# serviceberry3/weiner_slamit_v2

Hardware: AMD Instinct MI355X
Metric: frames/sec ORB extract+match @640x480x8lvl (higher is better)
Workload: dtype u8; 1 GPU; BASELINE configs[1]: 640x480 8-level ORB extract (1000 features, FAST 20/7) + brute-force 256-bit Hamming best/second match vs the stream's previous frame; 256 independent streams per GPU per step; distinct_frame_pairs_per_gpu=16, parallelism=streams sharded over 1 GPU(s), no data-path collective

## Files before the change

weiner_slamit_v2_amd/csrc/orb_kernels.hip:

```cpp
#include <hip/hip_runtime.h>
#include <stdint.h>

#include <algorithm>

#include "orb_types.h"
#include "slamit_math.h"
#include "../../include/slamit.h"
#include "../../include/slamit_orb_pattern.h"

#define WAVE 64

__global__ __launch_bounds__(256) void resize_level_kernel(
    const uint8_t* __restrict__ src, int sw, int sh, size_t sstride, size_t sframe,
    uint8_t* __restrict__ dst, int dw, int dh, size_t dstride, size_t dframe,
    const int* __restrict__ xofs, const short* __restrict__ ialpha,
    const int* __restrict__ yofs, const short* __restrict__ ibeta) {
    const int x4 = (blockIdx.x * 64 + (threadIdx.x & 63)) * 4;
    const int y = blockIdx.y * 4 + (threadIdx.x >> 6);
    const int f = blockIdx.z;
    if (x4 >= dw || y >= dh) return;
    const uint8_t* S = src + (size_t)f * sframe;
    int sy = yofs[y];
    int sy0 = min(max(sy, 0), sh - 1), sy1 = min(max(sy + 1, 0), sh - 1);
    const uint8_t* S0 = S + (size_t)sy0 * sstride;
// ... 752 lines not shown
            int lx = order & 63, ly = (order >> 6) & 63, cell = order >> 12;
            int ci = (int)__umulhi((unsigned)cell, inv_cols), cj = cell - ci * nCols;
            int x = cj * wCell + lx, y = ci * hCell + ly;
            int r = (int)((float)x / hX);
            r = min(r, nIni - 1);
            if (valid) XY[k] = (uint32_t)x | ((uint32_t)y << 16);
            if (FD) {
                Box16 b = box0[r];
                int path = 0;
                for (int d = 0; d < FD; ++d) {
                    int mx, my;
                    const int q = box_quadrant(b, x, y, &mx, &my);
                    b = child_box(b, q);
                    path = path * 4 + q;
                }
                if (valid) ND[k] = (uint16_t)((r << 8) | path);
                const int bin = valid ? r * HS + (HS - (1 << (2 * FD))) + path : -1;
                const int prev = __shfl_up(bin, 1);
                const bool head = lane == 0 || bin != prev;
                const unsigned long long heads = __ballot(head);
                if (head && bin >= 0) {
                    const unsigned long long rest = (heads >> lane) >> 1;
                    atomicAdd(&hist[bin], rest ? (int)__builtin_ctzll(rest) + 1 : 64 - lane);
                }
            } else {
                if (valid) ND[k] = (uint16_t)r;
                for (int q = 0; q < nIni; ++q) {
                    const unsigned long long m = __ballot(valid && r == q);
                    if (m && lane == (int)__builtin_ctzll(m)) atomicAdd(&cnt0[q], (int)__popcll(m));
                }
            }
            }
        }
    }
    __syncthreads();
    for (int d = FD - 1; d >= 1; --d) {
        const int off = ((4 << (2 * d)) - 4) / 3 - (1 << (2 * d)), offc = off + (1 << (2 * d)), per = 1 << (2 * d);
        for (int e = tid; e < nIni * per; e += NT) {
            const int r = e >> (2 * d), pth = e & (per - 1);
            const int* c = &hist[r * HS + offc + 4 * pth];
            hist[r * HS + off + pth] = (c[0] + c[1]) + (c[2] + c[3]);
        }
        __syncthreads();
    }
    if (tid == 0) {
        int m = 0, dropped = 0;
        for (int i = 0; i < nIni; ++i) {
            if (FD) cnt0[i] = (hist[i * HS] + hist[i * HS + 1]) + (hist[i * HS + 2] + hist[i * HS + 3]);
            if (cnt0[i] > 0) { scanbuf[i] = m; box0[m] = box0[i]; cnt0[m] = cnt0[i]; ncode0[m] = i << 16; ++m; }
            else { scanbuf[i] = -1; dropped = 1; }
        }
        s_n = m; s_flag = dropped;
    }
    __syncthreads();
    if (s_flag && !FD) {
        for (int k = tid; k < n_keys; k += NT) ND[k] = (uint16_t)scanbuf[ND[k]];
        __syncthreads();
    }

    int cur = 0;
    int n = s_n;
    bool finish = false, careful = false;
    bool tabled = FD > 0;
    int depth_done = 0;
    auto label_keys = [&]() {
        for (int e = tid; e < nIni * HS; e += NT) hist[e] = -1;
        if (tid < ORB_MAX_ROOTS) scanbuf[tid] = -1;
        __syncthreads();
        for (int i = tid; i < n; i += NT) {
            const int c = ncode0[cur * cap + i], r = c >> 16, d = (c >> 12) & 15, pth = c & 4095;
            if (d == 0) scanbuf[r] = i;
            else hist[r * HS + ((4 << (2 * d)) - 4) / 3 - (1 << (2 * d)) + pth] = i;
        }
        __syncthreads();
        for (int k = tid; k < n_keys; k += NT) {
            const int lab = ND[k], r = lab >> 8, pth = lab & 255;
            int node = scanbuf[r];
            for (int d = 1; d <= FD; ++d) {
                const int v = hist[r * HS + ((4 << (2 * d)) - 4) / 3 - (1 << (2 * d)) + (pth >> (2 * (FD - d)))];
                node = v >= 0 ? v : node;
            }
            ND[k] = (uint16_t)node;
        }
        __syncthreads();
    };
    OD_STAMP(0);
    while (!finish) {
        const int prevSize = n;
#ifdef OCT_DIAG
        ++od_pass;
#endif
        const bool tpass = tabled && !careful && depth_done < FD;
        if (tabled && !tpass) { label_keys(); tabled = false; }
        if (tpass) {
            for (int e = tid; e < 4 * n; e += NT) {
                const int i = e >> 2, c = ncode0[cur * cap + i], r = c >> 16, d = (c >> 12) & 15, pth = c & 4095;
                childcnt[e] = cnt0[cur * cap + i] > 1 ? hist[r * HS + ((4 << (2 * (d + 1))) - 4) / 3 - (1 << (2 * (d + 1))) + 4 * pth + (e & 3)] : 0;
            }
        } else {
        for (int i = tid; i < 4 * n; i += NT) childcnt[i] = 0;
        __syncthreads();
        for (int k = tid; k < n_keys; k += NT) {
            int nd = ND[k];
            if (cnt0[cur * cap + nd] > 1) {
                uint32_t xy = XY[k];
                int mx, my;
                int q = box_quadrant(box0[cur * cap + nd], xy & 0xFFFF, xy >> 16, &mx, &my);
                atomicAdd(&childcnt[nd * 4 + q], 1);
                ND[k] = (uint16_t)(nd | ((q + 1) << 12));
            }
        }
        }
        __syncthreads();
        OD_STAMP(1);

        int kproc;
        if (!careful) {
            kproc = -1;
        } else {
            for (int i = tid >> 6; i < n; i += NT / 64) {
                const int ci_ = cnt0[cur * cap + i];
                int r = -1;
                if (ci_ > 1) {
                    r = 0;
                    for (int j0 = 0; j0 < n; j0 += 64) {
                        const int j = j0 + (tid & 63);
                        const int cj_ = j < n ? cnt0[cur * cap + j] : 0;
                        r += (int)__popcll(__ballot((cj_ > 1) && (cj_ > ci_ || (cj_ == ci_ && j < i))));
                    }
                    if ((tid & 63) == 0) sorted[r] = i;
                }
                if ((tid & 63) == 0) rankv[i] = r;
            }
            if (tid == 0) s_expand = 0;
            __syncthreads();
            int local = 0;
            for (int i = tid; i < n; i += NT) local += cnt0[cur * cap + i] > 1;
            if (local) atomicAdd(&s_expand, local);
            __syncthreads();
            const int m = s_expand;
            for (int s = tid; s < m; s += NT) {
                int i = sorted[s];
                const int* cc = &childcnt[i * 4];
                scanbuf[s] = (cc[0] > 0) + (cc[1] > 0) + (cc[2] > 0) + (cc[3] > 0) - 1;
            }
            if (tid == 0) s_k = m;
            __syncthreads();
            block_exclusive_scan<NT>(scanbuf, m, wave_tmp);
            for (int s = tid; s < m; s += NT) {
                int i = sorted[s];
                const int* cc = &childcnt[i * 4];
                int g = (cc[0] > 0) + (cc[1] > 0) + (cc[2] > 0) + (cc[3] > 0) - 1;
                if (n + scanbuf[s] + g >= N) atomicMin(&s_k, s + 1);
            }
            __syncthreads();
            kproc = s_k;
        }

        OD_STAMP(2);
        int nchildslots;
        if (!careful) {
            nchildslots = 4 * n;
            for (int e = tid; e < 4 * n; e += NT) {
                int i = n - 1 - (e >> 2), q = 3 - (e & 3);
                scanbuf[e] = (cnt0[cur * cap + i] > 1) && (childcnt[i * 4 + q] > 0);
            }
            for (int i = tid; i < n; i += NT) scanbuf[4 * n + i] = cnt0[cur * cap + i] <= 1;
        } else {
            nchildslots = 4 * kproc;
            for (int e = tid; e < nchildslots; e += NT) {
                int s = kproc - 1 - (e >> 2), q = 3 - (e & 3);
                scanbuf[e] = childcnt[sorted[s] * 4 + q] > 0;
            }
            for (int i = tid; i < n; i += NT) {
                int r = rankv[i];
                scanbuf[nchildslots + i] = !(r >= 0 && r < kproc);
            }
        }
        __syncthreads();
        const int n_new = block_exclusive_scan<NT>(scanbuf, nchildslots + n, wave_tmp);
        const int nxt = cur ^ 1;
        if (tid == 0) s_expand = 0;
        __syncthreads();
        int local_expand = 0;
        for (int e = tid; e < nchildslots; e += NT) {
            int i, q;
            if (!careful) { i = n - 1 - (e >> 2); q = 3 - (e & 3); }
            else { i = sorted[kproc - 1 - (e >> 2)]; q = 3 - (e & 3); }
            bool split = !careful ? (cnt0[cur * cap + i] > 1) : true;
            int cc = childcnt[i * 4 + q];
            if (split && cc > 0) {
                int pos = scanbuf[e];
                if (pos < cap) {
                    box0[nxt * cap + pos] = child_box(box0[cur * cap + i], q);
                    cnt0[nxt * cap + pos] = cc;
                    if (tpass) { const int c = ncode0[cur * cap + i]; ncode0[nxt * cap + pos] = (c & ~0xFFFF) | ((((c >> 12) & 15) + 1) << 12) | (4 * (c & 4095) + q); }
                }
                local_expand += cc > 1;
            }
        }
        for (int i = tid; i < n; i += NT) {
            bool stays = !careful ? (cnt0[cur * cap + i] <= 1) : !(rankv[i] >= 0 && rankv[i] < kproc);
            if (stays) {
                int pos = scanbuf[nchildslots + i];
                if (pos < cap) {
                    box0[nxt * cap + pos] = box0[cur * cap + i]; cnt0[nxt * cap + pos] = cnt0[cur * cap + i];
                    if (tpass) ncode0[nxt * cap + pos] = ncode0[cur * cap + i];
                }
            }
        }
        if (local_expand) atomicAdd(&s_expand, local_expand);
        OD_STAMP(3);
        if (!tpass)
        for (int k = tid; k < n_keys; k += NT) {
            const int lab = ND[k];
            const int nd = lab & 4095, q = (lab >> 12) - 1;
            bool split = !careful ? (q >= 0) : (rankv[nd] >= 0 && rankv[nd] < kproc);
            int pos;
            if (split) {
                int e = !careful ? ((n - 1 - nd) * 4 + (3 - q)) : ((kproc - 1 - rankv[nd]) * 4 + (3 - q));
                pos = scanbuf[e];
            } else {
                pos = scanbuf[nchildslots + nd];
            }
            ND[k] = (uint16_t)min(pos, cap - 1);
        }
        __syncthreads();
        const int nToExpand = s_expand;
        cur = nxt;
        n = min(n_new, cap);
        __syncthreads();
        if (n >= N || n == prevSize) finish = true;
        else if (!careful && n + nToExpand * 3 > N) careful = true;
        ++depth_done;
        OD_STAMP(4);
    }
    if (tabled) label_keys();

    for (int i = tid; i < n; i += NT) best[i] = 0ull;
    __syncthreads();
    for (int k = tid; k < n_keys; k += NT) {
        unsigned long long c = K[k];
        unsigned long long packed = (c & 0xFFFFFFFF00000000ull) | (0xFFFFFFFFu - (unsigned)c);
        atomicMax(&best[ND[k]], packed);
    }
    __syncthreads();
    for (int i = tid; i < n; i += NT) {
        unsigned long long b = best[i];
        unsigned order = 0xFFFFFFFFu - (unsigned)b;
        int lx = order & 63, ly = (order >> 6) & 63, cell = order >> 12;
        int ci = cell / L.nCols, cj = cell - ci * L.nCols;
        OrbLevelKp kp;
        kp.x = (int16_t)(cj * L.wCell + lx + ORB_MIN_BORDER);
        kp.y = (int16_t)(ci * L.hCell + ly + ORB_MIN_BORDER);
        kp.response = (float)(unsigned)(b >> 32);
        kp.angle = 0.f; kp.cs = 1.f; kp.sn = 0.f;
        if (i < L.kp_cap) OUT[i] = kp;
    }
    if (tid == 0) *kp_count_out = min(n, L.kp_cap);
#ifdef OCT_DIAG
    OD_STAMP(5);
    if (tid == 0) {
        const int w = blockIdx.y * gridDim.x + blockIdx.x;
        if (w < 4096) { unsigned long long* o = g_oct_ph + 8 * w; for (int k = 0; k < 6; ++k) o[k] = od_ph[k]; o[6] = ((unsigned long long)od_pass << 32) | (unsigned)n_keys; o[7] = od_rt0; o[5] = __builtin_amdgcn_s_memrealtime(); }
    }
#endif
}

template <int OCT_NT>
__global__ __launch_bounds__(OCT_NT) void octree_kernel(
    const OrbLevel* __restrict__ levels, int nlevels,
    const unsigned long long* __restrict__ cand, size_t cand_frame_stride,
    int* __restrict__ cand_count,
    uint32_t* __restrict__ ws_xy, uint16_t* __restrict__ ws_node,
    OrbLevelKp* __restrict__ lkp, size_t kp_frame_stride, int* __restrict__ kp_count,
    int node_cap, int key_cap, int level_override ) {
    extern __shared__ __attribute__((aligned(16))) unsigned char smem[];
    __shared__ int wave_tmp[OCT_NT / 64];
    __shared__ int s_vars[4];
    uint32_t* k_xy = reinterpret_cast<uint32_t*>(smem + orbk_octree_node_bytes(node_cap));
    uint16_t* k_nd = reinterpret_cast<uint16_t*>(k_xy + key_cap);
    const int level = level_override >= 0 ? level_override : blockIdx.y;
    const int frame = blockIdx.x;
    const OrbLevel& L = levels[level];
    const int kidx = frame * nlevels + level;
    const int n_raw = cand_count[kidx * ORB_CC_PAD];
    const int n_keys = min(n_raw, L.cand_cap);
    __syncthreads();
    if (threadIdx.x == 0) { cand_count[kidx * ORB_CC_PAD] = 0; cand_count[kidx * ORB_CC_PAD + 1] = n_raw; }
    const unsigned long long* K = cand + L.cand_off + (size_t)frame * cand_frame_stride;
    OrbLevelKp* OUT = lkp + L.kp_off + (size_t)frame * kp_frame_stride;
    if (n_keys == 0) {
        if (threadIdx.x == 0) kp_count[kidx] = 0;
        return;
    }
    if (n_keys <= key_cap)
        octree_body<OCT_NT, true>(L, K, n_keys, k_xy, k_nd, OUT, &kp_count[kidx], smem, node_cap, wave_tmp, s_vars);
    else
        octree_body<OCT_NT, false>(L, K, n_keys, ws_xy + L.cand_off + (size_t)frame * cand_frame_stride,
                                        ws_node + L.cand_off + (size_t)frame * cand_frame_stride, OUT, &kp_count[kidx], smem,
                                        node_cap, wave_tmp, s_vars);
}

struct DiscTable { signed char uv[64][32]; int n; };
__constant__ DiscTable c_disc;

static DiscTable make_disc() {
    static const int umax[16] = {15, 15, 15, 15, 14, 14, 14, 13, 13, 12, 11, 10, 9, 8, 6, 3};
    DiscTable t;
    for (int l = 0; l < 64; ++l) for (int k = 0; k < 32; ++k) t.uv[l][k] = 0;
    t.n = 0;
    for (int v = -15; v <= 15; ++v)
        for (int u = -umax[v < 0 ? -v : v]; u <= umax[v < 0 ? -v : v]; ++u) {
            t.uv[t.n & 63][2 * (t.n >> 6)] = (signed char)u; t.uv[t.n & 63][2 * (t.n >> 6) + 1] = (signed char)v;
            ++t.n;
        }
    return t;
}

#define IC_KP_PER_WAVE 8
#define IC_R 15
#define IC_ROWS (2 * IC_R + 1)
#define IC_PITCH 32

template <int CTRL>
__device__ __forceinline__ int dpp_i32(int v) { return __builtin_amdgcn_update_dpp(0, v, CTRL, 0xF, 0xF, false); }
__device__ __forceinline__ int wave_sum_i32(int v) {
    v += dpp_i32<0xB1>(v);
    v += dpp_i32<0x4E>(v);
    v += dpp_i32<0x141>(v);
    v += dpp_i32<0x140>(v);
    return __builtin_amdgcn_readlane(v, 0) + __builtin_amdgcn_readlane(v, 16) + __builtin_amdgcn_readlane(v, 32) + __builtin_amdgcn_readlane(v, 48);
}

__global__ __launch_bounds__(256) void ic_angle_kernel(
    const OrbLevel* __restrict__ levels, int nlevels,
    const uint8_t* __restrict__ img0, size_t img0_stride, size_t img0_frame,
    const uint8_t* __restrict__ pyr,
    OrbLevelKp* __restrict__ lkp, size_t kp_frame_stride, const int* __restrict__ kp_count, int xcd_frames, int kblocks) {
    const int lane = threadIdx.x & 63;
    int level, frame, kb;
    if (xcd_frames) {
        const unsigned w = blockIdx.x, k = w >> 3, P = (unsigned)(nlevels * kblocks), fq = k / P, local = k - fq * P;
        frame = (int)(8u * fq + ((w + fq) & 7u));
        if (frame >= xcd_frames) return;
        level = (int)(local / (unsigned)kblocks); kb = (int)(local - (unsigned)level * (unsigned)kblocks);
    } else { level = blockIdx.y; frame = blockIdx.z; kb = blockIdx.x; }
    const OrbLevel& L = levels[level];
    const int count = kp_count[frame * nlevels + level];
    const int i0 = (kb * 4 + (threadIdx.x >> 6)) * IC_KP_PER_WAVE;
    if (i0 >= count) return;
    const uint8_t* src;
    int stride;
    if (level == 0) { src = img0 + (size_t)frame * img0_frame; stride = (int)img0_stride; }
    else { src = pyr + L.plane_off + (size_t)frame * L.plane_bytes; stride = L.stride; }
    __shared__ __attribute__((aligned(16))) uint8_t s_win[4][IC_KP_PER_WAVE][IC_ROWS * IC_PITCH];
    const int wvi = threadIdx.x >> 6;
    OrbLevelKp* kp0 = lkp + L.kp_off + (size_t)frame * kp_frame_stride;
    typedef unsigned ic_u4 __attribute__((ext_vector_type(4), aligned(1)));
    {
        const int lr = min(lane >> 1, IC_ROWS - 1), lc = lane & 1;
        const unsigned loff = __umul24((unsigned)lr, (unsigned)stride) + 16u * (unsigned)lc;
        ic_u4 ld[IC_KP_PER_WAVE];
#pragma unroll
        for (int k = 0; k < IC_KP_PER_WAVE; ++k) {
            const int i = min(i0 + k, count - 1);
            const uint8_t* corner = src + (__umul24((unsigned)(kp0[i].y - IC_R), (unsigned)stride) + (unsigned)(kp0[i].x - IC_R));
            ld[k] = *reinterpret_cast<const ic_u4*>(corner + loff);
        }
#pragma unroll
        for (int k = 0; k < IC_KP_PER_WAVE; ++k)
            if (lane < 2 * IC_ROWS) *reinterpret_cast<uint4*>(&s_win[wvi][k][lr * IC_PITCH + 16 * lc]) = make_uint4(ld[k].x, ld[k].y, ld[k].z, ld[k].w);
    }
    int off[12], wu[12], wv[12];
    {
        const uint4 t0 = *reinterpret_cast<const uint4*>(&c_disc.uv[lane][0]);
        const uint2 t1 = *reinterpret_cast<const uint2*>(&c_disc.uv[lane][16]);
        const uint32_t tw[6] = {t0.x, t0.y, t0.z, t0.w, t1.x, t1.y};
#pragma unroll
        for (int j = 0; j < 12; ++j) {
            const uint32_t pr = tw[j >> 1] >> (16 * (j & 1));
            const int u = (int)(signed char)(pr & 0xFFu), v = (int)(signed char)((pr >> 8) & 0xFFu);
            off[j] = (v + IC_R) * IC_PITCH + (u + IC_R); wu[j] = u; wv[j] = v;
        }
    }
    const float factorPI = (float)(3.14159265358979323846 / 180.f);
    wave_sync_lds();
    int val[IC_KP_PER_WAVE][12];
#pragma unroll
    for (int k = 0; k < IC_KP_PER_WAVE; ++k)
#pragma unroll
        for (int j = 0; j < 12; ++j) val[k][j] = s_win[wvi][k][off[j]];
    int V[2 * IC_KP_PER_WAVE];
#pragma unroll
    for (int k = 0; k < IC_KP_PER_WAVE; ++k) {
        int m10 = 0, m01 = 0;
#pragma unroll
        for (int j = 0; j < 12; ++j) { m10 += __mul24(wu[j], val[k][j]); m01 += __mul24(wv[j], val[k][j]); }
        V[2 * k] = m10; V[2 * k + 1] = m01;
    }
    {
        const bool b0 = lane & 1, b1 = lane & 2, b2 = lane & 4, b3 = lane & 8;
#pragma unroll
        for (int p = 0; p < 8; ++p) { const int a = V[2 * p], b = V[2 * p + 1]; V[p] = (b0 ? b : a) + dpp_i32<0xB1>(b0 ? a : b); }
#pragma unroll
        for (int p = 0; p < 4; ++p) { const int a = V[2 * p], b = V[2 * p + 1]; V[p] = (b1 ? b : a) + dpp_i32<0x4E>(b1 ? a : b); }
#pragma unroll
        for (int p = 0; p < 2; ++p) { const int a = V[2 * p], b = V[2 * p + 1]; V[p] = (b2 ? b : a) + dpp_i32<0x1B>(dpp_i32<0x141>(b2 ? a : b)); }
        { const int a = V[0], b = V[1]; V[0] = (b3 ? b : a) + dpp_i32<0x141>(dpp_i32<0x140>(b3 ? a : b)); }
    }
    __shared__ int s_rows[4][64];
    int* sr = s_rows[threadIdx.x >> 6];
    sr[lane] = V[0];
    wave_sync_lds();
    const int tot = (sr[lane & 15] + sr[(lane & 15) + 16]) + (sr[(lane & 15) + 32] + sr[(lane & 15) + 48]);
    const int my10 = tot, my01 = dpp_i32<0xB1>(tot);
    if (lane < 2 * IC_KP_PER_WAVE && !(lane & 1) && i0 + (lane >> 1) < count) {
        const float ang = slamit_fast_atan2((float)my01, (float)my10);
        float sn, cs;
        slamit_sincosf(ang * factorPI, &sn, &cs);
        OrbLevelKp* kp = kp0 + i0 + (lane >> 1);
        kp->angle = ang; kp->cs = cs; kp->sn = sn;
    }
}

__device__ __forceinline__ int reflect101(int p, int len) {
    p = p < 0 ? -p : p;
    p = p >= len ? 2 * len - 2 - p : p;
    return min(max(p, 0), len - 1);
}


typedef unsigned short blur_us2 __attribute__((ext_vector_type(2)));
__device__ __forceinline__ uint32_t udot2(uint32_t a, uint32_t b, uint32_t c) {
    return __builtin_amdgcn_udot2(__builtin_bit_cast(blur_us2, a), __builtin_bit_cast(blur_us2, b), c, false);
}

__device__ __forceinline__ uint32_t blur_fetch(const uint8_t* S, unsigned sstride, bool whole, int w, int h, int gx0, int row) {
    const unsigned ro = (unsigned)reflect101(row, h) * sstride;
    if (whole) return *reinterpret_cast<const uint32_t*>(S + (ro + (unsigned)gx0));
    if (gx0 >= w + 3) return 0u;
    uint32_t v = 0;
#pragma unroll
    for (int j = 0; j < 4; ++j) v |= (uint32_t)S[ro + (unsigned)reflect101(gx0 + j, w)] << (8 * j);
    return v;
}

struct BlurCol { unsigned a0, a1, sel; };
__device__ __forceinline__ BlurCol blur_col(int g, int w, unsigned ss) {
#define BLUR_SEL(i0, i1, i2, i3) ((unsigned)(i0) | ((unsigned)(i1) << 8) | ((unsigned)(i2) << 16) | ((unsigned)(i3) << 24))
    BlurCol c;
    if (g < 0) { c.a0 = 0u; c.a1 = 4u; c.sel = BLUR_SEL(4, 3, 2, 1); }
    else if (g + 4 <= w) { c.a0 = c.a1 = (unsigned)g; c.sel = BLUR_SEL(0, 1, 2, 3); }
    else if (g < w) {
        const int q = w - g;
        unsigned idx[4];
#pragma unroll
        for (int j = 0; j < 4; ++j) idx[j] = (unsigned)(j < q ? 4 + j : 2 * q + 2 - j);
        c.a0 = (unsigned)(g - 4); c.a1 = (unsigned)g; c.sel = BLUR_SEL(idx[0], idx[1], idx[2], idx[3]);
    } else if (g <= w + 2) {
        const int t = g - w, gb = (w - 4) & ~3;
        unsigned idx[4];
#pragma unroll
        for (int j = 0; j < 4; ++j) idx[j] = j <= 2 - t ? (unsigned)(w - 2 - t - j - gb) : 0x0Cu;
        c.a0 = (unsigned)gb; c.a1 = min((unsigned)gb + 4u, ss - 4u); c.sel = BLUR_SEL(idx[0], idx[1], idx[2], idx[3]);
    } else { c.a0 = c.a1 = 0u; c.sel = BLUR_SEL(0x0C, 0x0C, 0x0C, 0x0C); }
#undef BLUR_SEL
    return c;
}
__device__ __forceinline__ uint32_t blur_fetch2(const uint8_t* S, unsigned ss, int h, int row, const BlurCol c) {
    const unsigned ro = __umul24((unsigned)reflect101(row, h), ss);
    return __builtin_amdgcn_perm(*reinterpret_cast<const uint32_t*>(S + (ro + c.a1)), *reinterpret_cast<const uint32_t*>(S + (ro + c.a0)), c.sel);
}

template <bool INTERIOR>
__device__ __forceinline__ void blur_strip(uint8_t (*in)[72], uint32_t (*rp)[64], const uint8_t* S, const size_t sstride, const bool aligned,
                                           uint8_t* D, const unsigned dstride, const int w, const int h, const int bx, const int by0, const int tid) {
    const int i0 = tid, i1 = tid + 256;
    const bool has1 = i1 < 22 * 18;
    const int r0 = i0 / 18, r1 = i1 / 18;
    const int g0 = bx - 4 + 4 * (i0 - r0 * 18), g1 = bx - 4 + 4 * (i1 - r1 * 18);
    const bool whole0 = aligned && g0 >= 0 && g0 + 4 <= w, whole1 = aligned && g1 >= 0 && g1 + 4 <= w;
    uint32_t* const st0 = reinterpret_cast<uint32_t*>(&in[r0][4 * (i0 - r0 * 18)]);
    uint32_t* const st1 = reinterpret_cast<uint32_t*>(&in[has1 ? r1 : 0][has1 ? 4 * (i1 - r1 * 18) : 0]);
    const unsigned ss = (unsigned)sstride;
    const BlurCol bc0 = blur_col(g0, w, ss), bc1 = blur_col(g1, w, ss);
    uint32_t v0 = INTERIOR ? *reinterpret_cast<const uint32_t*>(S + (__umul24((unsigned)(by0 + r0 - 3), ss) + (unsigned)g0))
                           : aligned ? blur_fetch2(S, ss, h, by0 + r0 - 3, bc0) : blur_fetch(S, ss, whole0, w, h, g0, by0 + r0 - 3);
    uint32_t v1 = !has1 ? 0u : INTERIOR ? *reinterpret_cast<const uint32_t*>(S + (__umul24((unsigned)(by0 + r1 - 3), ss) + (unsigned)g1))
                                        : aligned ? blur_fetch2(S, ss, h, by0 + r1 - 3, bc1) : blur_fetch(S, ss, whole1, w, h, g1, by0 + r1 - 3);
    *st0 = v0;
    if (has1) *st1 = v1;
    __syncthreads();
    const uint32_t TA = 18u | (34u << 8) | (49u << 16) | (55u << 24), TB = 49u | (34u << 8) | (18u << 16);
    const int cy = tid >> 4, cx4 = (tid & 15) * 4;
    const bool odd = cy & 1;
    const uint32_t k0 = odd ? (18u << 16) : (18u | (34u << 16)), k1 = odd ? (34u | (49u << 16)) : (49u | (55u << 16));
    const uint32_t k2 = odd ? (55u | (49u << 16)) : (49u | (34u << 16)), k3 = odd ? (34u | (18u << 16)) : 18u;
#pragma unroll 1
    for (int s = 0; s < BLUR_STEPS; ++s) {
        const int by = by0 + 16 * s;
        const bool more = s + 1 < BLUR_STEPS && (INTERIOR || by + 16 < h);
        if (more) {
            if (INTERIOR) {
                v0 = *reinterpret_cast<const uint32_t*>(S + (__umul24((unsigned)(by + 16 + r0 - 3), ss) + (unsigned)g0));
                if (has1) v1 = *reinterpret_cast<const uint32_t*>(S + (__umul24((unsigned)(by + 16 + r1 - 3), ss) + (unsigned)g1));
            } else {
                if (aligned) {
                    v0 = blur_fetch2(S, ss, h, by + 16 + r0 - 3, bc0);
                    if (has1) v1 = blur_fetch2(S, ss, h, by + 16 + r1 - 3, bc1);
                } else {
                    v0 = blur_fetch(S, ss, whole0, w, h, g0, by + 16 + r0 - 3);
                    if (has1) v1 = blur_fetch(S, ss, whole1, w, h, g1, by + 16 + r1 - 3);
                }
            }
        }
        if (tid < 11 * 16) {
            const int p = tid >> 4, c = (tid & 15) * 4;
            uint32_t o[2][4];
#pragma unroll
            for (int rr = 0; rr < 2; ++rr) {
                const uint32_t* pw = reinterpret_cast<const uint32_t*>(&in[2 * p + rr][c]);
                const uint32_t w0 = pw[0], w1 = pw[1], w2 = pw[2];
                o[rr][0] = __builtin_amdgcn_udot4(__builtin_amdgcn_alignbyte(w2, w1, 1), TB, __builtin_amdgcn_udot4(__builtin_amdgcn_alignbyte(w1, w0, 1), TA, 0u, false), false);
                o[rr][1] = __builtin_amdgcn_udot4(__builtin_amdgcn_alignbyte(w2, w1, 2), TB, __builtin_amdgcn_udot4(__builtin_amdgcn_alignbyte(w1, w0, 2), TA, 0u, false), false);
                o[rr][2] = __builtin_amdgcn_udot4(__builtin_amdgcn_alignbyte(w2, w1, 3), TB, __builtin_amdgcn_udot4(__builtin_amdgcn_alignbyte(w1, w0, 3), TA, 0u, false), false);
                o[rr][3] = __builtin_amdgcn_udot4(w2, TB, __builtin_amdgcn_udot4(w1, TA, 0u, false), false);
            }
            *reinterpret_cast<uint4*>(&rp[p][c]) = make_uint4(o[0][0] | (o[1][0] << 16), o[0][1] | (o[1][1] << 16),
                                                               o[0][2] | (o[1][2] << 16), o[0][3] | (o[1][3] << 16));
        }
        __syncthreads();
        if (more) {
            *st0 = v0;
            if (has1) *st1 = v1;
        }
        if (INTERIOR || (bx + cx4 < w && by + cy < h)) {
            const int pb = cy >> 1;
            const uint4 a0 = *reinterpret_cast<const uint4*>(&rp[pb][cx4]), a1 = *reinterpret_cast<const uint4*>(&rp[pb + 1][cx4]);
            const uint4 a2 = *reinterpret_cast<const uint4*>(&rp[pb + 2][cx4]), a3 = *reinterpret_cast<const uint4*>(&rp[pb + 3][cx4]);
#define BLUR_COL(f) min((udot2(a3.f, k3, udot2(a2.f, k2, udot2(a1.f, k1, udot2(a0.f, k0, 1u << 15)))) >> 16), 255u)
            const uint32_t out = BLUR_COL(x) | (BLUR_COL(y) << 8) | (BLUR_COL(z) << 16) | (BLUR_COL(w) << 24);
#undef BLUR_COL
            *reinterpret_cast<uint32_t*>(D + (__umul24((unsigned)(by + cy), dstride) + (unsigned)(bx + cx4))) = out;
        }
        if (!more) break;
        __syncthreads();
    }
}

__global__ __launch_bounds__(256) void blur_all_kernel(
    const OrbLevel* __restrict__ levels, const uint4* __restrict__ tiles,
    const uint8_t* __restrict__ img0, size_t img0_stride, size_t img0_frame,
    const uint8_t* __restrict__ pyr, uint8_t* __restrict__ blur, unsigned ntiles, unsigned inv_tiles, unsigned total) {
    __shared__ __attribute__((aligned(16))) uint8_t in[22][72];
    __shared__ __attribute__((aligned(16))) uint32_t rp[11][64];
    const int tid = threadIdx.x;
    const unsigned lin = blockIdx.x, per_xcd = (total + 7u) >> 3;
    const unsigned logical = (lin & 7u) * per_xcd + (lin >> 3);
    if (logical >= total) return;
    int frame = (int)__umulhi(logical, inv_tiles);
    if ((unsigned)frame * ntiles > logical) --frame;
    const uint4 tt = tiles[logical - (unsigned)frame * ntiles];
    const int level = (int)tt.x, bx = (int)tt.y, by0 = (int)tt.z;
    const OrbLevel& L = levels[level];
    const int w = L.w, h = L.h;
    const uint8_t* S;
    size_t sstride;
    if (level == 0) { S = img0 + (size_t)frame * img0_frame; sstride = img0_stride; }
    else { S = pyr + L.plane_off + (size_t)frame * L.plane_bytes; sstride = (size_t)L.stride; }
    const bool aligned = ((((uintptr_t)S) | sstride) & 3) == 0;
    uint8_t* D = blur + L.blur_off + (size_t)frame * L.blur_bytes;
    const bool interior = aligned && bx >= 4 && bx + 68 <= w && by0 >= 3 && by0 + ORB_BLUR_STRIP_H + 3 <= h;
    if (interior) blur_strip<true>(in, rp, S, sstride, aligned, D, (unsigned)L.stride, w, h, bx, by0, tid);
    else blur_strip<false>(in, rp, S, sstride, aligned, D, (unsigned)L.stride, w, h, bx, by0, tid);
}

template <bool EDGE>
__global__ __launch_bounds__(256) void blur_stream_kernel(
    const OrbLevel* __restrict__ levels, const uint4* __restrict__ tiles,
    const uint8_t* __restrict__ img0, size_t img0_stride, size_t img0_frame,
    const uint8_t* __restrict__ pyr, uint8_t* __restrict__ blur, unsigned ntiles) {
    const unsigned tile = blockIdx.x * 16u + (threadIdx.x >> 4);
    if (tile >= ntiles) return;
    const int frame = blockIdx.y;
    const uint4 tt = tiles[tile];
    const int level = (int)tt.x, by0 = (int)tt.z;
    const int x0 = (int)tt.y + 4 * (int)(threadIdx.x & 15);
    const OrbLevel& L = levels[level];
    const int h = L.h;
    const uint8_t* S;
    unsigned ss;
    if (level == 0) { S = img0 + (size_t)frame * img0_frame; ss = (unsigned)img0_stride; }
    else { S = pyr + L.plane_off + (size_t)frame * L.plane_bytes; ss = (unsigned)L.stride; }
    if (EDGE && x0 >= L.w) return;
    BlurCol bc[3];
    if (EDGE) {
#pragma unroll
        for (int k = 0; k < 3; ++k) bc[k] = blur_col(x0 - 4 + 4 * k, L.w, ss);
    } else S += x0 - 4;
    uint8_t* D = blur + L.blur_off + (size_t)frame * L.blur_bytes + x0;
    const unsigned ds = (unsigned)L.stride;
    const uint32_t TA = 18u | (34u << 8) | (49u << 16) | (55u << 24), TB = 49u | (34u << 8) | (18u << 16);
    const uint32_t kA0 = 18u | (34u << 16), kA1 = 49u | (55u << 16), kA2 = 49u | (34u << 16), kA3 = 18u;
    const uint32_t kB0 = 18u << 16, kB1 = 34u | (49u << 16), kB2 = 55u | (49u << 16), kB3 = 34u | (18u << 16);
    const int ylast = min(by0 + ORB_BLUR_STRIP_H, h) - 1;
    const int p0 = (by0 - 3) >> 1, p1 = (ylast + 3) >> 1;
    typedef unsigned blur_u3 __attribute__((ext_vector_type(3)));
    auto fetch = [&](int yy) -> blur_u3 {
        int r = yy < 0 ? -yy : yy;
        r = r >= h ? 2 * h - 2 - r : r;
        r = min(max(r, 0), h - 1);
        if (EDGE) {
            const uint8_t* R = S + __umul24((unsigned)r, ss);
            blur_u3 v;
            v.x = __builtin_amdgcn_perm(*reinterpret_cast<const uint32_t*>(R + bc[0].a1), *reinterpret_cast<const uint32_t*>(R + bc[0].a0), bc[0].sel);
            v.y = __builtin_amdgcn_perm(*reinterpret_cast<const uint32_t*>(R + bc[1].a1), *reinterpret_cast<const uint32_t*>(R + bc[1].a0), bc[1].sel);
            v.z = __builtin_amdgcn_perm(*reinterpret_cast<const uint32_t*>(R + bc[2].a1), *reinterpret_cast<const uint32_t*>(R + bc[2].a0), bc[2].sel);
            return v;
        }
        return *reinterpret_cast<const blur_u3*>(S + __umul24((unsigned)r, ss));
    };
    auto rowpass = [&](const blur_u3 v, uint32_t* o) {
        o[0] = __builtin_amdgcn_udot4(__builtin_amdgcn_alignbyte(v.z, v.y, 1), TB, __builtin_amdgcn_udot4(__builtin_amdgcn_alignbyte(v.y, v.x, 1), TA, 0u, false), false);
        o[1] = __builtin_amdgcn_udot4(__builtin_amdgcn_alignbyte(v.z, v.y, 2), TB, __builtin_amdgcn_udot4(__builtin_amdgcn_alignbyte(v.y, v.x, 2), TA, 0u, false), false);
        o[2] = __builtin_amdgcn_udot4(__builtin_amdgcn_alignbyte(v.z, v.y, 3), TB, __builtin_amdgcn_udot4(__builtin_amdgcn_alignbyte(v.y, v.x, 3), TA, 0u, false), false);
        o[3] = __builtin_amdgcn_udot4(v.z, TB, __builtin_amdgcn_udot4(v.y, TA, 0u, false), false);
    };
    uint32_t P0[4] = {0, 0, 0, 0}, P1[4] = {0, 0, 0, 0}, P2[4] = {0, 0, 0, 0}, P3[4];
    blur_u3 va = fetch(2 * p0), vb = fetch(2 * p0 + 1), va1 = fetch(2 * p0 + 2), vb1 = fetch(2 * p0 + 3), va2 = fetch(2 * p0 + 4), vb2 = fetch(2 * p0 + 5);
#pragma unroll 4
    for (int p = p0; p <= p1; ++p) {
        const blur_u3 ca = va, cb = vb;
        va = va1; vb = vb1; va1 = va2; vb1 = vb2;
        va2 = fetch(2 * p + 6); vb2 = fetch(2 * p + 7);
        uint32_t oa[4], ob[4];
        rowpass(ca, oa); rowpass(cb, ob);
#pragma unroll
        for (int j = 0; j < 4; ++j) P3[j] = oa[j] | (ob[j] << 16);
        const int ya = 2 * p - 3, yb = 2 * p - 2;
#define BLUR_OUT(k0, k1, k2, k3, j) min((udot2(P3[j], k3, udot2(P2[j], k2, udot2(P1[j], k1, udot2(P0[j], k0, 1u << 15)))) >> 16), 255u)
        if (ya >= by0 && ya <= ylast)
            *reinterpret_cast<uint32_t*>(D + __umul24((unsigned)ya, ds)) = BLUR_OUT(kA0, kA1, kA2, kA3, 0) | (BLUR_OUT(kA0, kA1, kA2, kA3, 1) << 8) | (BLUR_OUT(kA0, kA1, kA2, kA3, 2) << 16) | (BLUR_OUT(kA0, kA1, kA2, kA3, 3) << 24);
        if (yb >= by0 && yb <= ylast)
            *reinterpret_cast<uint32_t*>(D + __umul24((unsigned)yb, ds)) = BLUR_OUT(kB0, kB1, kB2, kB3, 0) | (BLUR_OUT(kB0, kB1, kB2, kB3, 1) << 8) | (BLUR_OUT(kB0, kB1, kB2, kB3, 2) << 16) | (BLUR_OUT(kB0, kB1, kB2, kB3, 3) << 24);
#undef BLUR_OUT
#pragma unroll
        for (int j = 0; j < 4; ++j) { P0[j] = P1[j]; P1[j] = P2[j]; P2[j] = P3[j]; }
    }
}

__constant__ __attribute__((aligned(16))) signed char c_pattern[SLAMIT_ORB_PATTERN_INTS];
#define DESC_KP_PER_WAVE 4
#define DESC_R 18
#define DESC_ROWS (2 * DESC_R + 1)
#define DESC_PITCH 48
#define DESC_LOADS 2

__global__ __launch_bounds__(256) void describe_kernel(
    const OrbLevel* __restrict__ levels, int nlevels,
    const uint8_t* __restrict__ blur,
    const OrbLevelKp* __restrict__ lkp, size_t kp_frame_stride, const int* __restrict__ kp_count,
    slamit_kp* __restrict__ out_kps, uint8_t* __restrict__ out_desc, int out_cap,
    int* __restrict__ out_n, int xcd_frames , int kblocks) {
    const int lane = threadIdx.x & 63;
    int level, frame, kb;
    if (xcd_frames) {
        const unsigned w = blockIdx.x, k = w >> 3, P = (unsigned)(nlevels * kblocks), fq = k / P, local = k - fq * P;
        frame = (int)(8u * fq + ((w + fq) & 7u));
        if (frame >= xcd_frames) return;
        level = (int)(local / (unsigned)kblocks); kb = (int)(local - (unsigned)level * (unsigned)kblocks);
    } else { level = blockIdx.y; frame = blockIdx.z; kb = blockIdx.x; }
    const int i0 = (kb * 4 + (threadIdx.x >> 6)) * DESC_KP_PER_WAVE;
    const OrbLevel& L = levels[level];
    const int* counts = kp_count + frame * nlevels;
    int offset = 0, total = 0;
    for (int l = 0; l < nlevels; ++l) {
        int c = counts[l];
        if (l < level) offset += c;
        total += c;
    }
    if (level == 0 && i0 == 0 && lane == 0) out_n[frame] = min(total, out_cap);
    const int count = counts[level];
    if (i0 >= count) return;
    const int4 pw = reinterpret_cast<const int4*>(c_pattern)[lane];
    const int pt[4] = {pw.x, pw.y, pw.z, pw.w};
    float px0[4], py0[4], px1[4], py1[4];
#pragma unroll
    for (int t = 0; t < 4; ++t) {
        px0[t] = (float)(signed char)(pt[t] & 0xFF); py0[t] = (float)(signed char)((pt[t] >> 8) & 0xFF);
        px1[t] = (float)(signed char)((pt[t] >> 16) & 0xFF); py1[t] = (float)(signed char)((pt[t] >> 24) & 0xFF);
    }
    const uint8_t* img = blur + L.blur_off + (size_t)frame * L.blur_bytes;
    const unsigned step = (unsigned)L.stride;
    const OrbLevelKp* KP = lkp + L.kp_off + (size_t)frame * kp_frame_stride;
    OrbLevelKp kp[DESC_KP_PER_WAVE];
#pragma unroll
    for (int k = 0; k < DESC_KP_PER_WAVE; ++k) kp[k] = KP[min(i0 + k, count - 1)];
    __shared__ __attribute__((aligned(16))) uint8_t s_patch[4][DESC_KP_PER_WAVE][DESC_ROWS * DESC_PITCH];
    const int wv = threadIdx.x >> 6;
    int lrow[DESC_LOADS], lcol[DESC_LOADS];
    unsigned poff[DESC_LOADS];
#pragma unroll
    for (int it = 0; it < DESC_LOADS; ++it) {
        const int idx = lane + 64 * it;
        lrow[it] = (int)(((unsigned)idx * 21846u) >> 16);
        lcol[it] = idx - 3 * lrow[it];
        poff[it] = __umul24((unsigned)min(lrow[it], DESC_ROWS - 1), step) + 16u * (unsigned)lcol[it];
    }
    const __amdgpu_buffer_rsrc_t rsrc = __builtin_amdgcn_make_buffer_rsrc(const_cast<uint8_t*>(img), 0, (unsigned)L.stride * (unsigned)L.h, 0x00020000);
    typedef unsigned desc_u4 __attribute__((ext_vector_type(4)));
    desc_u4 ld[DESC_KP_PER_WAVE][DESC_LOADS];
#pragma unroll
    for (int k = 0; k < DESC_KP_PER_WAVE; ++k) {
        const unsigned base = __umul24((unsigned)(kp[k].y - DESC_R), step) + (unsigned)((kp[k].x - DESC_R) & ~3);
#pragma unroll
        for (int it = 0; it < DESC_LOADS; ++it) ld[k][it] = __builtin_amdgcn_raw_buffer_load_b128(rsrc, (int)(base + poff[it]), 0, 0);
    }
#pragma unroll
    for (int k = 0; k < DESC_KP_PER_WAVE; ++k)
#pragma unroll
        for (int it = 0; it < DESC_LOADS; ++it)
            if (lrow[it] < DESC_ROWS) *reinterpret_cast<desc_u4*>(&s_patch[wv][k][__mul24(lrow[it], DESC_PITCH) + 16 * lcol[it]]) = ld[k][it];
    __builtin_amdgcn_fence(__ATOMIC_ACQ_REL, "wavefront");
    __builtin_amdgcn_wave_barrier();
    typedef float desc_f2 __attribute__((ext_vector_type(2)));
    const desc_f2 magic = {12582912.0f, 12582912.0f};
    const unsigned DESC_BIAS = 0x400000u * (unsigned)DESC_PITCH + 0x4B400000u;
    int tv0[DESC_KP_PER_WAVE][4], tv1[DESC_KP_PER_WAVE][4];
#pragma unroll
    for (int k = 0; k < DESC_KP_PER_WAVE; ++k) {
        const float a = kp[k].cs, b = kp[k].sn;
        const desc_f2 ba = {b, a}, anb = {a, -b};
        const uint8_t* center = &s_patch[wv][k][DESC_R * DESC_PITCH + DESC_R + ((kp[k].x - DESC_R) & 3)];
        const uint8_t* biased = center - DESC_BIAS;
#pragma unroll
        for (int t = 0; t < 4; ++t) {
            const desc_f2 p0 = {px0[t], px0[t]}, q0 = {py0[t], py0[t]}, p1 = {px1[t], px1[t]}, q1 = {py1[t], py1[t]};
            const desc_f2 m0 = (p0 * ba + q0 * anb) + magic, m1 = (p1 * ba + q1 * anb) + magic;
            tv0[k][t] = biased[__umul24(__float_as_uint(m0.x), (unsigned)DESC_PITCH) + __float_as_uint(m0.y)];
            tv1[k][t] = biased[__umul24(__float_as_uint(m1.x), (unsigned)DESC_PITCH) + __float_as_uint(m1.y)];
        }
    }
#pragma unroll
    for (int k = 0; k < DESC_KP_PER_WAVE; ++k) {
        const int i = i0 + k, o = offset + i;
        unsigned nib = 0;
#pragma unroll
        for (int t = 0; t < 4; ++t) nib |= (unsigned)(tv0[k][t] < tv1[k][t]) << t;
        unsigned other = __shfl_xor(nib, 1, WAVE);
        if (i >= count || o >= out_cap) continue;
        if ((lane & 1) == 0)
            out_desc[((size_t)frame * out_cap + o) * SLAMIT_DESC_BYTES + (lane >> 1)] = (uint8_t)(nib | (other << 4));
        if (lane == 0) {
            slamit_kp kk;
            float fx = (float)kp[k].x, fy = (float)kp[k].y;
            if (level != 0) { fx *= L.scale; fy *= L.scale; }
            kk.x = fx; kk.y = fy; kk.size = L.patch_size; kk.angle = kp[k].angle; kk.response = kp[k].response;
            kk.octave = level; kk.class_id = -1;
            out_kps[(size_t)frame * out_cap + o] = kk;
        }
    }
}

__global__ __launch_bounds__(256) void pad_level_kernel(const uint8_t* __restrict__ src, int w, int h,
                                                        size_t sstride, uint8_t* __restrict__ dst) {
    const int B = SLAMIT_EDGE_THRESHOLD;
    const int pw = w + 2 * B, ph = h + 2 * B;
    int x = blockIdx.x * 64 + (threadIdx.x & 63), y = blockIdx.y * 4 + (threadIdx.x >> 6);
    if (x >= pw || y >= ph) return;
    dst[(size_t)y * pw + x] = src[(size_t)reflect101(y - B, h) * sstride + reflect101(x - B, w)];
}

__global__ void decode_candidates_kernel(const OrbLevel* __restrict__ levels, int level,
                                         const unsigned long long* __restrict__ K, int n,
                                         unsigned long long* __restrict__ order_out, int* __restrict__ xys) {
    int k = blockIdx.x * blockDim.x + threadIdx.x;
    if (k >= n) return;
    const OrbLevel& L = levels[level];
    unsigned long long c = K[k];
    unsigned order = (unsigned)c;
    int lx = order & 63, ly = (order >> 6) & 63, cell = order >> 12;
    int ci = cell / L.nCols, cj = cell - ci * L.nCols;
    xys[3 * k + 0] = cj * L.wCell + lx;
    xys[3 * k + 1] = ci * L.hCell + ly;
    xys[3 * k + 2] = (int)(c >> 32);
    order_out[k] = order;
}

extern "C++" {

hipError_t orbk_upload_pattern(hipStream_t st) {
    static const DiscTable disc = make_disc();
    hipError_t e = hipMemcpyToSymbolAsync(HIP_SYMBOL(c_disc), &disc, sizeof(disc), 0, hipMemcpyHostToDevice, st);
    if (e != hipSuccess) return e;
    return hipMemcpyToSymbolAsync(HIP_SYMBOL(c_pattern), slamit_orb_pattern, SLAMIT_ORB_PATTERN_INTS, 0,
                                  hipMemcpyHostToDevice, st);
}

void orbk_resize(hipStream_t st, const uint8_t* src, int sw, int sh, size_t sstride, size_t sframe,
                 uint8_t* dst, int dw, int dh, size_t dstride, size_t dframe, const int* xofs,
                 const short* ialpha, const int* yofs, const short* ibeta, int nframes) {
    dim3 grid((dw + 255) / 256, (dh + 3) / 4, nframes);
    hipLaunchKernelGGL(resize_level_kernel, grid, dim3(256), 0, st, src, sw, sh, sstride, sframe, dst, dw,
                       dh, dstride, dframe, xofs, ialpha, yofs, ibeta);
}

hipError_t orbk_pyramid_prepare(int smem_bytes) {
    return hipFuncSetAttribute(reinterpret_cast<const void*>(pyramid_fused_kernel),
                               hipFuncAttributeMaxDynamicSharedMemorySize, smem_bytes);
}

void orbk_pyramid(hipStream_t st, const OrbLevel* levels, int nlevels, const PyrBox* boxes, const PyrTabs* tabs,
                  int nregions, const uint8_t* img0, size_t img0_stride, size_t img0_frame, uint8_t* pyr, int bufA_bytes,
                  int smem_bytes, int nframes, int l_first, int l_last) {
    hipLaunchKernelGGL(pyramid_fused_kernel, dim3(nregions, nframes), dim3(PYR_THREADS), smem_bytes, st, levels, nlevels, boxes,
                       tabs, img0, img0_stride, img0_frame, pyr, bufA_bytes, l_first, l_last);
}

#ifndef FAST_PS
#define FAST_PS 48
#define FAST_PL 80
#endif
static int fast_pitch(int max_wcell) { return max_wcell + 11 <= FAST_PS ? FAST_PS : FAST_PL; }

size_t orbk_fast_smem(int max_wcell, int max_hcell) {
    const int P = fast_pitch(max_wcell);
    const int tile_rows = max_hcell + 6, sc_rows = max_hcell + 2;
    const int kp_cap = ((max_wcell + 1) / 2) * ((max_hcell + 1) / 2);
    return (size_t)4 * fast_wave_bytes(P, tile_rows, sc_rows, kp_cap);
}

hipError_t orbk_fast_prepare(int max_wcell, int max_hcell) {
    const int smem = (int)orbk_fast_smem(max_wcell, max_hcell);
    hipError_t e;
    if (fast_pitch(max_wcell) == FAST_PS) {
        e = hipFuncSetAttribute(reinterpret_cast<const void*>(fast_cells_kernel<FAST_PS>), hipFuncAttributeMaxDynamicSharedMemorySize, smem);
    } else {
        e = hipFuncSetAttribute(reinterpret_cast<const void*>(fast_cells_kernel<FAST_PL>), hipFuncAttributeMaxDynamicSharedMemorySize, smem);
    }
    return e;
}

void orbk_fast(hipStream_t st, const FastTab& tab, int nlevels, const uint32_t* d_cells, int cells_per_frame,
               const uint8_t* img0, size_t img0_stride, size_t img0_frame, const uint8_t* pyr,
               unsigned long long* cand, size_t cand_frame_stride, int* cand_count, int iniTh, int minTh,
               int max_wcell, int max_hcell, int nframes) {
    const int tile_rows = max_hcell + 6, sc_rows = max_hcell + 2;
    const int kp_cap = ((max_wcell + 1) / 2) * ((max_hcell + 1) / 2);
    const int wpb = cells_per_frame < 1600 ? 1 : 4;
    const int xcd_frames = nframes >= 16 ? nframes : 0;
    const dim3 grid = xcd_frames ? dim3((unsigned)(((nframes + 7) / 8) * 8) * (unsigned)((cells_per_frame + wpb - 1) / wpb))
                                 : dim3(wpb == 1 ? (unsigned)((cells_per_frame + 31) & ~31) : (unsigned)((cells_per_frame + wpb - 1) / wpb), nframes);
    const size_t smem = orbk_fast_smem(max_wcell, max_hcell) / 4 * wpb;
    if (fast_pitch(max_wcell) == FAST_PS)
        hipLaunchKernelGGL(fast_cells_kernel<FAST_PS>, grid, dim3(64 * wpb), smem, st, tab, reinterpret_cast<const uint4*>(d_cells), nlevels, cells_per_frame, img0,
                           (unsigned)img0_stride, img0_frame, pyr, cand, cand_frame_stride, cand_count, iniTh, minTh, tile_rows,
                           sc_rows, kp_cap, xcd_frames);
    else
        hipLaunchKernelGGL(fast_cells_kernel<FAST_PL>, grid, dim3(64 * wpb), smem, st, tab, reinterpret_cast<const uint4*>(d_cells), nlevels, cells_per_frame, img0,
                           (unsigned)img0_stride, img0_frame, pyr, cand, cand_frame_stride, cand_count, iniTh, minTh, tile_rows,
                           sc_rows, kp_cap, xcd_frames);
}

hipError_t orbk_octree_prepare(int node_cap, int key_cap) {
    static int prepared = 0;
    const int want = (int)orbk_octree_smem(node_cap, key_cap);
    if (want <= prepared) return hipSuccess;
    prepared = want;
    hipError_t e = hipFuncSetAttribute(reinterpret_cast<const void*>(octree_kernel<256>), hipFuncAttributeMaxDynamicSharedMemorySize, want);
    if (e != hipSuccess) return e;
    e = hipFuncSetAttribute(reinterpret_cast<const void*>(octree_kernel<OCT_THREADS>), hipFuncAttributeMaxDynamicSharedMemorySize, want);
    if (e != hipSuccess) return e;
    return hipFuncSetAttribute(reinterpret_cast<const void*>(octree_kernel<1024>), hipFuncAttributeMaxDynamicSharedMemorySize, want);
}

void orbk_octree(hipStream_t st, const OrbLevel* levels, int nlevels, const unsigned long long* cand,
                 size_t cand_frame_stride, int* cand_count, uint32_t* ws_xy, uint16_t* ws_node,
                 OrbLevelKp* lkp, size_t kp_frame_stride, int* kp_count, int node_cap, int key_cap, int nframes,
                 int level_override) {
    dim3 grid(nframes, level_override >= 0 ? 1 : nlevels);
    const int nt = nframes >= 96 ? 256 : nframes <= 16 ? 1024 : OCT_THREADS;
    if (nframes >= 96) key_cap = std::min(key_cap, 2048);
    if (nt == 1024)
        hipLaunchKernelGGL(octree_kernel<1024>, grid, dim3(1024), orbk_octree_smem(node_cap, key_cap), st, levels, nlevels, cand,
                           cand_frame_stride, cand_count, ws_xy, ws_node, lkp, kp_frame_stride, kp_count, node_cap,
                           key_cap, level_override);
    else if (nt == 256)
        hipLaunchKernelGGL(octree_kernel<256>, grid, dim3(256), orbk_octree_smem(node_cap, key_cap), st, levels, nlevels, cand,
                           cand_frame_stride, cand_count, ws_xy, ws_node, lkp, kp_frame_stride, kp_count, node_cap,
                           key_cap, level_override);
    else
        hipLaunchKernelGGL(octree_kernel<OCT_THREADS>, grid, dim3(OCT_THREADS), orbk_octree_smem(node_cap, key_cap), st, levels, nlevels, cand,
                           cand_frame_stride, cand_count, ws_xy, ws_node, lkp, kp_frame_stride, kp_count, node_cap,
                           key_cap, level_override);
}

void orbk_ic_angle(hipStream_t st, const OrbLevel* levels, int nlevels, const uint8_t* img0,
                   size_t img0_stride, size_t img0_frame, const uint8_t* pyr, OrbLevelKp* lkp,
                   size_t kp_frame_stride, const int* kp_count, int max_kp, int nframes) {
    const int kblocks = (max_kp + 4 * IC_KP_PER_WAVE - 1) / (4 * IC_KP_PER_WAVE);
    if (nframes >= 16)
        hipLaunchKernelGGL(ic_angle_kernel, dim3((unsigned)(((nframes + 7) / 8) * 8 * nlevels * kblocks)), dim3(256), 0, st, levels,
                           nlevels, img0, img0_stride, img0_frame, pyr, lkp, kp_frame_stride, kp_count, nframes, kblocks);
    else
        hipLaunchKernelGGL(ic_angle_kernel, dim3(kblocks, nlevels, nframes), dim3(256), 0, st, levels,
                           nlevels, img0, img0_stride, img0_frame, pyr, lkp, kp_frame_stride, kp_count, 0, kblocks);
}

void orbk_blur_stream(hipStream_t st, const OrbLevel* levels, const uint32_t* d_tiles, int ntiles, const uint8_t* img0,
                      size_t img0_stride, size_t img0_frame, const uint8_t* pyr, uint8_t* blur, int nframes, bool edge) {
    if (ntiles <= 0) return;
    if (edge)
        hipLaunchKernelGGL(blur_stream_kernel<true>, dim3((ntiles + 15) / 16, nframes), dim3(256), 0, st, levels, reinterpret_cast<const uint4*>(d_tiles), img0,
                           img0_stride, img0_frame, pyr, blur, (unsigned)ntiles);
    else
        hipLaunchKernelGGL(blur_stream_kernel<false>, dim3((ntiles + 15) / 16, nframes), dim3(256), 0, st, levels, reinterpret_cast<const uint4*>(d_tiles), img0,
                           img0_stride, img0_frame, pyr, blur, (unsigned)ntiles);
}

void orbk_blur(hipStream_t st, const OrbLevel* levels, const uint32_t* d_tiles, int total_tiles, const uint8_t* img0,
               size_t img0_stride, size_t img0_frame, const uint8_t* pyr, uint8_t* blur, int nframes) {
    if (total_tiles <= 0) return;
    const unsigned total = (unsigned)total_tiles * (unsigned)nframes, grid = ((total + 7u) >> 3) << 3;
    const unsigned inv = (unsigned)((0x100000000ull + (unsigned)total_tiles - 1) / (unsigned)total_tiles);
    hipLaunchKernelGGL(blur_all_kernel, dim3(grid), dim3(256), 0, st, levels, reinterpret_cast<const uint4*>(d_tiles), img0,
                       img0_stride, img0_frame, pyr, blur, (unsigned)total_tiles, inv, total);
}

void orbk_describe(hipStream_t st, const OrbLevel* levels, int nlevels, const uint8_t* blur,
                   const OrbLevelKp* lkp, size_t kp_frame_stride, const int* kp_count, slamit_kp* out_kps,
                   uint8_t* out_desc, int out_cap, int* out_n, int max_kp, int nframes) {
    const int kblocks = (max_kp + 4 * DESC_KP_PER_WAVE - 1) / (4 * DESC_KP_PER_WAVE);
    if (nframes >= 16)
        hipLaunchKernelGGL(describe_kernel, dim3((unsigned)(((nframes + 7) / 8) * 8 * nlevels * kblocks)), dim3(256), 0, st, levels,
                           nlevels, blur, lkp, kp_frame_stride, kp_count, out_kps, out_desc, out_cap, out_n, nframes, kblocks);
    else
        hipLaunchKernelGGL(describe_kernel, dim3(kblocks, nlevels, nframes), dim3(256), 0, st, levels,
                           nlevels, blur, lkp, kp_frame_stride, kp_count, out_kps, out_desc, out_cap, out_n, 0, kblocks);
}

void orbk_pad(hipStream_t st, const uint8_t* src, int w, int h, size_t sstride, uint8_t* dst) {
    hipLaunchKernelGGL(pad_level_kernel, dim3((w + 38 + 63) / 64, (h + 38 + 3) / 4), dim3(256), 0, st, src, w, h,
                       sstride, dst);
}

void orbk_decode_candidates(hipStream_t st, const OrbLevel* levels, int level, const unsigned long long* K,
                            int n, unsigned long long* order_out, int* xys) {
    if (n <= 0) return;
    hipLaunchKernelGGL(decode_candidates_kernel, dim3((n + 255) / 256), dim3(256), 0, st, levels, level, K, n,
                       order_out, xys);
}

}
```

Baseline: 305,300 frames/s.

## Compute IC angle moments with udot4 masks directly from registers, skipping LDS

Rewrites the intensity-centroid angle computation. Each lane already holds a 16-byte row segment of the patch, so it now takes the disc-masked row sum and the column-weighted sum with packed u8 dot products (udot4) against per-lane mask and weight tables. m10 and m01 are then derived algebraically from those sums, which removes the shared-memory window staging, the wave LDS sync, and the 12 scattered LDS reads plus multiply-adds per keypoint. The mask table and the fixed row/column lane mapping must reproduce the original disc exactly.

Measured after the change: 305,800 frames/s, median of 6. About the same (+0.2%).

```diff
diff --git a/weiner_slamit_v2_amd/csrc/orb_kernels.hip b/weiner_slamit_v2_amd/csrc/orb_kernels.hip
--- a/weiner_slamit_v2_amd/csrc/orb_kernels.hip
+++ b/weiner_slamit_v2_amd/csrc/orb_kernels.hip
@@ -1078,26 +1078,30 @@
                                         node_cap, wave_tmp, s_vars);
 }
 
-struct DiscTable { signed char uv[64][32]; int n; };
-__constant__ DiscTable c_disc;
-
-static DiscTable make_disc() {
+struct IcMaskTable { uint32_t m[64][8]; };
+__constant__ __attribute__((aligned(16))) IcMaskTable c_icmask;
+
+static IcMaskTable make_icmask() {
     static const int umax[16] = {15, 15, 15, 15, 14, 14, 14, 13, 13, 12, 11, 10, 9, 8, 6, 3};
-    DiscTable t;
-    for (int l = 0; l < 64; ++l) for (int k = 0; k < 32; ++k) t.uv[l][k] = 0;
-    t.n = 0;
-    for (int v = -15; v <= 15; ++v)
-        for (int u = -umax[v < 0 ? -v : v]; u <= umax[v < 0 ? -v : v]; ++u) {
-            t.uv[t.n & 63][2 * (t.n >> 6)] = (signed char)u; t.uv[t.n & 63][2 * (t.n >> 6) + 1] = (signed char)v;
-            ++t.n;
-        }
+    IcMaskTable t;
+    for (int l = 0; l < 64; ++l) {
+        for (int k = 0; k < 8; ++k) t.m[l][k] = 0;
+        const int r = l >> 1, c = l & 1;
+        if (r > 30) continue;
+        const int v = r - 15, um = umax[v < 0 ? -v : v];
+        for (int b = 0; b < 16; ++b) {
+            const int col = 16 * c + b, u = col - 15;
+            if (u < -um || u > um) continue;
+            t.m[l][b >> 2] |= 1u << (8 * (b & 3));
+            t.m[l][4 + (b >> 2)] |= (uint32_t)col << (8 * (b & 3));
+        }
+    }
     return t;
 }
 
 #define IC_KP_PER_WAVE 8
 #define IC_R 15
 #define IC_ROWS (2 * IC_R + 1)
-#define IC_PITCH 32
 
 template <int CTRL>
 __device__ __forceinline__ int dpp_i32(int v) { return __builtin_amdgcn_update_dpp(0, v, CTRL, 0xF, 0xF, false); }
@@ -1130,50 +1134,30 @@
     int stride;
     if (level == 0) { src = img0 + (size_t)frame * img0_frame; stride = (int)img0_stride; }
     else { src = pyr + L.plane_off + (size_t)frame * L.plane_bytes; stride = L.stride; }
-    __shared__ __attribute__((aligned(16))) uint8_t s_win[4][IC_KP_PER_WAVE][IC_ROWS * IC_PITCH];
-    const int wvi = threadIdx.x >> 6;
     OrbLevelKp* kp0 = lkp + L.kp_off + (size_t)frame * kp_frame_stride;
     typedef unsigned ic_u4 __attribute__((ext_vector_type(4), aligned(1)));
-    {
-        const int lr = min(lane >> 1, IC_ROWS - 1), lc = lane & 1;
-        const unsigned loff = __umul24((unsigned)lr, (unsigned)stride) + 16u * (unsigned)lc;
-        ic_u4 ld[IC_KP_PER_WAVE];
-#pragma unroll
-        for (int k = 0; k < IC_KP_PER_WAVE; ++k) {
-            const int i = min(i0 + k, count - 1);
-            const uint8_t* corner = src + (__umul24((unsigned)(kp0[i].y - IC_R), (unsigned)stride) + (unsigned)(kp0[i].x - IC_R));
-            ld[k] = *reinterpret_cast<const ic_u4*>(corner + loff);
-        }
-#pragma unroll
-        for (int k = 0; k < IC_KP_PER_WAVE; ++k)
-            if (lane < 2 * IC_ROWS) *reinterpret_cast<uint4*>(&s_win[wvi][k][lr * IC_PITCH + 16 * lc]) = make_uint4(ld[k].x, ld[k].y, ld[k].z, ld[k].w);
-    }
-    int off[12], wu[12], wv[12];
-    {
-        const uint4 t0 = *reinterpret_cast<const uint4*>(&c_disc.uv[lane][0]);
-        const uint2 t1 = *reinterpret_cast<const uint2*>(&c_disc.uv[lane][16]);
-        const uint32_t tw[6] = {t0.x, t0.y, t0.z, t0.w, t1.x, t1.y};
-#pragma unroll
-        for (int j = 0; j < 12; ++j) {
-            const uint32_t pr = tw[j >> 1] >> (16 * (j & 1));
-            const int u = (int)(signed char)(pr & 0xFFu), v = (int)(signed char)((pr >> 8) & 0xFFu);
-            off[j] = (v + IC_R) * IC_PITCH + (u + IC_R); wu[j] = u; wv[j] = v;
-        }
+    const int lr = min(lane >> 1, IC_ROWS - 1), lc = lane & 1;
+    const unsigned loff = __umul24((unsigned)lr, (unsigned)stride) + 16u * (unsigned)lc;
+    const int vrow = lr - IC_R;
+    const uint4 mk = *reinterpret_cast<const uint4*>(&c_icmask.m[lane][0]);
+    const uint4 wt = *reinterpret_cast<const uint4*>(&c_icmask.m[lane][4]);
+    ic_u4 ld[IC_KP_PER_WAVE];
+#pragma unroll
+    for (int k = 0; k < IC_KP_PER_WAVE; ++k) {
+        const int i = min(i0 + k, count - 1);
+        const uint8_t* corner = src + (__umul24((unsigned)(kp0[i].y - IC_R), (unsigned)stride) + (unsigned)(kp0[i].x - IC_R));
+        ld[k] = *reinterpret_cast<const ic_u4*>(corner + loff);
     }
     const float factorPI = (float)(3.14159265358979323846 / 180.f);
-    wave_sync_lds();
-    int val[IC_KP_PER_WAVE][12];
-#pragma unroll
-    for (int k = 0; k < IC_KP_PER_WAVE; ++k)
-#pragma unroll
-        for (int j = 0; j < 12; ++j) val[k][j] = s_win[wvi][k][off[j]];
     int V[2 * IC_KP_PER_WAVE];
 #pragma unroll
     for (int k = 0; k < IC_KP_PER_WAVE; ++k) {
-        int m10 = 0, m01 = 0;
-#pragma unroll
-        for (int j = 0; j < 12; ++j) { m10 += __mul24(wu[j], val[k][j]); m01 += __mul24(wv[j], val[k][j]); }
-        V[2 * k] = m10; V[2 * k + 1] = m01;
+        const unsigned s0 = __builtin_amdgcn_udot4(ld[k].w, mk.w, __builtin_amdgcn_udot4(ld[k].z, mk.z,
+                            __builtin_amdgcn_udot4(ld[k].y, mk.y, __builtin_amdgcn_udot4(ld[k].x, mk.x, 0u, false), false), false), false);
+        const unsigned s1 = __builtin_amdgcn_udot4(ld[k].w, wt.w, __builtin_amdgcn_udot4(ld[k].z, wt.z,
+                            __builtin_amdgcn_udot4(ld[k].y, wt.y, __builtin_amdgcn_udot4(ld[k].x, wt.x, 0u, false), false), false), false);
+        V[2 * k] = (int)s1 - IC_R * (int)s0;
+        V[2 * k + 1] = vrow * (int)s0;
     }
     {
         const bool b0 = lane & 1, b1 = lane & 2, b2 = lane & 4, b3 = lane & 8;
@@ -1567,8 +1551,8 @@
 extern "C++" {
 
 hipError_t orbk_upload_pattern(hipStream_t st) {
-    static const DiscTable disc = make_disc();
-    hipError_t e = hipMemcpyToSymbolAsync(HIP_SYMBOL(c_disc), &disc, sizeof(disc), 0, hipMemcpyHostToDevice, st);
+    static const IcMaskTable icmask = make_icmask();
+    hipError_t e = hipMemcpyToSymbolAsync(HIP_SYMBOL(c_icmask), &icmask, sizeof(icmask), 0, hipMemcpyHostToDevice, st);
     if (e != hipSuccess) return e;
     return hipMemcpyToSymbolAsync(HIP_SYMBOL(c_pattern), slamit_orb_pattern, SLAMIT_ORB_PATTERN_INTS, 0,
                                   hipMemcpyHostToDevice, st);
```
